# AOS55/exorl

Measured on AMD Instinct MI355X. Metric: gradient-steps/sec TD3+BC walker_walk batch=1024, higher is better.
Workload: dtype bf16x3

## Files before the change

exorl_amd/csrc/fused.hip:

```cpp
#include "kernels.h"

namespace exorl {

constexpr int MAX_IN = 256;
constexpr float LN_EPS2 = 1e-5f;

constexpr int TF_ROWS = 8;
constexpr int TF_LDS_FLOATS = 35 * 1024;

__device__ __forceinline__ float tanh_fast(float x) {
    const float e = __expf(2.0f * x);
    return 1.0f - 2.0f * __frcp_rn(1.0f + e);
}

template <bool FAST>
__global__ __launch_bounds__(512) void trunk_fwd_kernel(const float* __restrict__ x, int64_t ldx,
                                                        const float* __restrict__ W0T, const float* __restrict__ b0,
                                                        const float* __restrict__ gain, const float* __restrict__ beta,
                                                        float* __restrict__ h, float* __restrict__ xhat,
                                                        float* __restrict__ rstd, unsigned short* __restrict__ hb,
                                                        unsigned short* __restrict__ xhb, int rows, int in_dim, int H,
                                                        int64_t astride, int64_t pstride, int64_t tstride, int TF_KC) {
    extern __shared__ __attribute__((aligned(16))) float smem[];
    float* ws = smem;
// ... 956 lines not shown
        float4 v;
        v.x = av.x > 0.f ? sacc.x : 0.f; v.y = av.y > 0.f ? sacc.y : 0.f;
        v.z = av.z > 0.f ? sacc.z : 0.f; v.w = av.w > 0.f ? sacc.w : 0.f;
        if (dz) reinterpret_cast<float4*>(dz + o)[c4] = v;
        if (dzb) reinterpret_cast<ushort4*>(dzb + o)[c4] = bf16_bits4(v);
        if (dzl) reinterpret_cast<ushort4*>(dzl + o)[c4] = bf16_lo_bits4(v);
        pb.x += v.x; pb.y += v.y; pb.z += v.z; pb.w += v.w;
    }
    if (want_params) {
#pragma unroll
        for (int j = 0; j < NO; ++j)
            if (j < nout) reinterpret_cast<float4*>(Pn + (int64_t)j * H)[c4] = pw[j];
        reinterpret_cast<float4*>(Pn + (int64_t)nout * H)[c4] = pb;
    }
}

int head_bwd(const DoutSpec& dspec, const float* W, const float* a, float* dz, const Planes& dzq, float* P, int rows,
             int H, int nout, int nets, int64_t astride, int64_t pstride, int want_params, hipStream_t s, bool metrics) {
    unsigned short *dz_bf16 = dzq.hi, *dz_lo = dzq.lo;
    EXORL_REQUIRE(nout >= 1 && nout <= 16 && H % 4 == 0 && H <= 1024, "head_bwd: nout=%d H=%d unsupported", nout, H);
    dim3 grid(cdiv(rows, HB_ROWS), nets);
    if (metrics) {
        EXORL_REQUIRE(dspec.mode == EXORL_DOUT_ACTOR_MU && dspec.kind == EXORL_AGENT_TD3_BC && nets == 1 && dspec.bc_part,
                      "head_bwd: the metrics variant is TD3+BC's actor gradient on one net");
        if (nout == 1) hipLaunchKernelGGL((head_bwd_kernel<1, true>), grid, dim3(256), 0, s, dspec, W, a, dz, dz_bf16, P, rows, H, nout, astride, pstride, want_params, dz_lo);
        else if (nout <= 8) hipLaunchKernelGGL((head_bwd_kernel<8, true>), grid, dim3(256), 0, s, dspec, W, a, dz, dz_bf16, P, rows, H, nout, astride, pstride, want_params, dz_lo);
        else hipLaunchKernelGGL((head_bwd_kernel<16, true>), grid, dim3(256), 0, s, dspec, W, a, dz, dz_bf16, P, rows, H, nout, astride, pstride, want_params, dz_lo);
    } else if (nout == 1) hipLaunchKernelGGL((head_bwd_kernel<1>), grid, dim3(256), 0, s, dspec, W, a, dz, dz_bf16, P, rows, H, nout, astride, pstride, want_params, dz_lo);
    else if (nout <= 8) hipLaunchKernelGGL((head_bwd_kernel<8>), grid, dim3(256), 0, s, dspec, W, a, dz, dz_bf16, P, rows, H, nout, astride, pstride, want_params, dz_lo);
    else hipLaunchKernelGGL((head_bwd_kernel<16>), grid, dim3(256), 0, s, dspec, W, a, dz, dz_bf16, P, rows, H, nout, astride, pstride, want_params, dz_lo);
    EXORL_LAUNCH_CHECK();
    return 0;
}
__global__ __launch_bounds__(256) void head_bwd_wide_kernel(const DoutSpec dspec, const float* __restrict__ W,
                                                            const float* __restrict__ a, float* __restrict__ dz,
                                                            unsigned short* __restrict__ dzb, float* __restrict__ P, int rows, int H,
                                                            int nout, int64_t astride, int64_t pstride, int want_params,
                                                            unsigned short* __restrict__ dzl) {
    __shared__ float ds[HB_ROWS * 32];
    const int net = blockIdx.z;
    const int row0 = blockIdx.y * HB_ROWS;
    const int c = blockIdx.x * 256 + threadIdx.x;
    {
        const int r = threadIdx.x >> 5, j = threadIdx.x & 31;
        ds[threadIdx.x] = (row0 + r < rows && j < nout) ? dout_value(dspec, net, row0 + r, j, rows, nout) : 0.f;
    }
    __syncthreads();
    const int64_t nh = (int64_t)(nout + 1) * H + 32;
    float* Pn = P ? P + ((int64_t)net * gridDim.y + blockIdx.y) * nh : nullptr;
    if (want_params && blockIdx.x == 0 && threadIdx.x < nout) {
        float sj = 0.f;
        for (int r = 0; r < HB_ROWS; ++r) sj += ds[r * 32 + threadIdx.x];
        Pn[(int64_t)(nout + 1) * H + threadIdx.x] = sj;
    }
    if (c >= H) return;
    float w[32], pw[32];
#pragma unroll
    for (int j = 0; j < 32; ++j) {
        w[j] = j < nout ? W[net * pstride + (int64_t)j * H + c] : 0.f;
        pw[j] = 0.f;
    }
    float pb = 0.f;
    const int nr = rows - row0 < HB_ROWS ? rows - row0 : HB_ROWS;
    for (int r = 0; r < nr; ++r) {
        const int64_t o = net * astride + (int64_t)(row0 + r) * H + c;
        const float av = a[o];
        float sacc = 0.f;
#pragma unroll
        for (int j = 0; j < 32; ++j) {
            const float d = ds[r * 32 + j];
            sacc += d * w[j];
            pw[j] += d * av;
        }
        const float v = av > 0.f ? sacc : 0.f;
        if (dz) dz[o] = v;
        if (dzb) dzb[o] = bf16_bits(v);
        if (dzl) dzl[o] = bf16_lo_bits(v);
        pb += v;
    }
    if (want_params) {
#pragma unroll
        for (int j = 0; j < 32; ++j)
            if (j < nout) Pn[(int64_t)j * H + c] = pw[j];
        Pn[(int64_t)nout * H + c] = pb;
    }
}

int head_bwd_wide(const DoutSpec& dspec, const float* W, const float* a, float* dz, const Planes& dzq, float* P, int rows, int H,
                  int nout, int64_t astride, int64_t pstride, int want_params, hipStream_t s) {
    unsigned short *dz_bf16 = dzq.hi, *dz_lo = dzq.lo;
    EXORL_REQUIRE(nout > 16 && nout <= 32, "head_bwd_wide: nout=%d out of range", nout);
    hipLaunchKernelGGL(head_bwd_wide_kernel, dim3(cdiv(H, 256), cdiv(rows, HB_ROWS), 1), dim3(256), 0, s, dspec, W, a, dz, dz_bf16, P, rows,
                       H, nout, astride, pstride, want_params, dz_lo);
    EXORL_LAUNCH_CHECK();
    return 0;
}

int head_chunks(int rows) { return cdiv(rows, HB_ROWS); }

constexpr int QH_ROWS = 4;
template <int MODE, bool TP, bool MET = false>
__global__ __launch_bounds__(256) void qhead_kernel(const QHeadArgs g) {
    __shared__ float part[4][4 * QH_ROWS];
    __shared__ float dq[2 * QH_ROWS];
    __shared__ float met[6 * QH_ROWS];
    const int row0 = blockIdx.x * QH_ROWS;
    const int c4 = threadIdx.x, H = g.H, H4 = H >> 2;
    const int lane = threadIdx.x & 63, wave = threadIdx.x >> 6;
    const int nr = g.rows - row0 < QH_ROWS ? g.rows - row0 : QH_ROWS;
    constexpr int nn = (MODE == 0 && !TP) ? 4 : 2;
    const bool on = c4 < H4;
    float4 avs[2][QH_ROWS];
    float4 w[2];
    float dots[4 * QH_ROWS];
    float4 wvs[nn], ts[nn][QH_ROWS];
    {
        const int cc = on ? c4 : 0;
#pragma unroll
        for (int n = 0; n < nn; ++n) {
            wvs[n] = reinterpret_cast<const float4*>(g.W[n])[cc];
#pragma unroll
            for (int r = 0; r < QH_ROWS; ++r) ts[n][r] = reinterpret_cast<const float4*>(g.a[n] + (int64_t)(row0 + (r < nr ? r : 0)) * H)[cc];
        }
    }
#pragma unroll
    for (int n = 0; n < 4; ++n) {
        if (n >= nn) {
#pragma unroll
            for (int r = 0; r < QH_ROWS; ++r) dots[n * QH_ROWS + r] = 0.f;
            continue;
        }
        const float4 wv = on ? wvs[n < nn ? n : 0] : make_float4(0.f, 0.f, 0.f, 0.f);
        if (n < 2) w[n] = wv;
#pragma unroll
        for (int r = 0; r < QH_ROWS; ++r) {
            const float4 t = (on && r < nr) ? ts[n < nn ? n : 0][r] : make_float4(0.f, 0.f, 0.f, 0.f);
            dots[n * QH_ROWS + r] = (t.x * wv.x + t.y * wv.y) + (t.z * wv.z + t.w * wv.w);
            if (n < 2) avs[n][r] = t;
        }
    }
#pragma unroll
    for (int i = 0; i < 4 * QH_ROWS; ++i) {
        const float v = wave_sum(dots[i]);
        if (lane == 0) part[wave][i] = v;
    }
    __syncthreads();
    if (threadIdx.x < 4 * QH_ROWS) {
        const int n = threadIdx.x / QH_ROWS, r = threadIdx.x % QH_ROWS;
        if (n < nn && r < nr) {
            const float v = ((part[0][threadIdx.x] + part[1][threadIdx.x]) + (part[2][threadIdx.x] + part[3][threadIdx.x])) + g.b[n][0];
            part[0][threadIdx.x] = v;
            (n < 2 ? g.q : g.tq)[(int64_t)(n & 1) * g.rows + row0 + r] = v;
        } else if (TP && MODE == 0 && n >= 2 && r < nr) {
            const float* tp = g.tpart[n - 2] + (int64_t)(row0 + r) * g.tslots;
            float v = 0.f;
            for (int j = 0; j < g.tslots; ++j) v += tp[j];
            v += g.b[n][0];
            part[0][threadIdx.x] = v;
            g.tq[(int64_t)(n & 1) * g.rows + row0 + r] = v;
        }
    }
    __syncthreads();
    if (threadIdx.x < 2 * QH_ROWS) {
        const int n = threadIdx.x / QH_ROWS, r = threadIdx.x % QH_ROWS;
        float d = 0.f, m_r = 0.f, m_y = 0.f, m_q = 0.f, m_e = 0.f;
        if (r < nr) {
            const float q1 = part[0][r], q2 = part[0][QH_ROWS + r];
            if (MODE == 0) {
                const float rw = g.reward[row0 + r];
                const float y = rw + g.discount[row0 + r] * fminf(part[0][2 * QH_ROWS + r], part[0][3 * QH_ROWS + r]);
                d = 2.0f * ((n == 0 ? q1 : q2) - y) * g.inv_bg;
                m_r = rw; m_y = y; m_q = n == 0 ? q1 : q2; m_e = (m_q - y) * (m_q - y);
            } else {
                const float w1 = q1 < q2 ? 1.0f : (q1 == q2 ? 0.5f : 0.0f);
                d = -g.inv_bg * (n == 0 ? w1 : 1.0f - w1);
            }
        }
        dq[threadIdx.x] = d;
        if (MODE == 0 && MET) {
            if (n == 0) { met[r] = m_r; met[QH_ROWS + r] = m_y; }
            met[(2 + n) * QH_ROWS + r] = m_q;
            met[(4 + n) * QH_ROWS + r] = m_e;
        }
    }
    if (MODE == 1 && threadIdx.x == 0) {
        float sa = 0.f, sm = 0.f;
        for (int r = 0; r < nr; ++r) { const float m = fminf(part[0][r], part[0][QH_ROWS + r]); sa += fabsf(m); sm += m; }
        g.abs_part[2 * blockIdx.x] = sa;
        g.abs_part[2 * blockIdx.x + 1] = sm;
    }
    __syncthreads();
    if (MODE == 0 && MET && threadIdx.x < 6) {
        float sk = 0.f;
        for (int r = 0; r < QH_ROWS; ++r) sk += met[threadIdx.x * QH_ROWS + r];
        g.abs_part[6 * blockIdx.x + threadIdx.x] = sk;
    }
    const int64_t nh = 2 * (int64_t)H + 16;
#pragma unroll
    for (int n = 0; n < 2; ++n) {
        float* Pn = g.P ? g.P + ((int64_t)n * gridDim.x + blockIdx.x) * nh : nullptr;
        if (Pn && threadIdx.x == 0) {
            float sj = 0.f;
            for (int r = 0; r < QH_ROWS; ++r) sj += dq[n * QH_ROWS + r];
            Pn[2 * (int64_t)H] = sj;
        }
        if (!on) continue;
        float4 pw = make_float4(0.f, 0.f, 0.f, 0.f), pb = make_float4(0.f, 0.f, 0.f, 0.f);
#pragma unroll
        for (int r = 0; r < QH_ROWS; ++r) {
            if (r >= nr) break;
            const float d = dq[n * QH_ROWS + r];
            const float4 av = avs[n][r];
            pw.x += d * av.x; pw.y += d * av.y; pw.z += d * av.z; pw.w += d * av.w;
            float4 v;
            v.x = av.x > 0.f ? d * w[n].x : 0.f; v.y = av.y > 0.f ? d * w[n].y : 0.f;
            v.z = av.z > 0.f ? d * w[n].z : 0.f; v.w = av.w > 0.f ? d * w[n].w : 0.f;
            const int64_t o = n * g.act + (int64_t)(row0 + r) * H;
            if (g.dz) reinterpret_cast<float4*>(g.dz + o)[c4] = v;
            if (g.dzb) reinterpret_cast<ushort4*>(g.dzb + o)[c4] = bf16_bits4(v);
            if (g.dzl) reinterpret_cast<ushort4*>(g.dzl + o)[c4] = bf16_lo_bits4(v);
            pb.x += v.x; pb.y += v.y; pb.z += v.z; pb.w += v.w;
        }
        if (Pn) {
            reinterpret_cast<float4*>(Pn)[c4] = pw;
            reinterpret_cast<float4*>(Pn + H)[c4] = pb;
        }
    }
}

int qhead_chunks(int rows) { return cdiv(rows, QH_ROWS); }

int qhead(const QHeadArgs& q, hipStream_t s, bool metrics) {
    EXORL_REQUIRE(q.H % 4 == 0 && q.H <= 1024 && q.rows > 0 && (q.mode == 0 || q.mode == 1), "qhead: unsupported H=%d rows=%d", q.H, q.rows);
    if (q.mode == 0 && metrics && q.tpart[0]) hipLaunchKernelGGL((qhead_kernel<0, true, true>), dim3(cdiv(q.rows, QH_ROWS)), dim3(256), 0, s, q);
    else if (q.mode == 0 && metrics) hipLaunchKernelGGL((qhead_kernel<0, false, true>), dim3(cdiv(q.rows, QH_ROWS)), dim3(256), 0, s, q);
    else if (q.mode == 0 && q.tpart[0]) hipLaunchKernelGGL((qhead_kernel<0, true>), dim3(cdiv(q.rows, QH_ROWS)), dim3(256), 0, s, q);
    else if (q.mode == 0) hipLaunchKernelGGL((qhead_kernel<0, false>), dim3(cdiv(q.rows, QH_ROWS)), dim3(256), 0, s, q);
    else hipLaunchKernelGGL((qhead_kernel<1, false>), dim3(cdiv(q.rows, QH_ROWS)), dim3(256), 0, s, q);
    EXORL_LAUNCH_CHECK();
    return 0;
}

__global__ __launch_bounds__(256) void finalize_grads_kernel(FinalizeArgs f) {
    const int H = f.H;
    const int64_t nh = (int64_t)(f.nout + 1) * H + (f.nout > 16 ? 32 : 16);
    const int64_t nt = 3 * (int64_t)H;
    const int64_t nw = (int64_t)f.in_dim * H;
    const int64_t total = f.n_heads * nh + f.n_trunks * (nt + nw);
    for (int64_t i = blockIdx.x * (int64_t)blockDim.x + threadIdx.x; i < total; i += (int64_t)gridDim.x * blockDim.x) {
        if (i < f.n_heads * nh) {
            const int net = (int)(i / nh);
            const int64_t e = i % nh;
            const int64_t j = e / H;
            if (j > f.nout && e - (int64_t)(f.nout + 1) * H >= f.nout) continue;
            const float sacc = chunk_sum(f.Ph + (int64_t)net * f.head_chunks * nh + e, f.head_chunks, nh);
            float* Gn = f.G + net * f.head_stride;
            if (j < f.nout) Gn[f.gW2 + e] = sacc;
            else if (j == f.nout) Gn[f.gb1 + (e - (int64_t)f.nout * H)] = sacc;
            else Gn[f.gb2 + (e - (int64_t)(f.nout + 1) * H)] = sacc;
        } else {
            const int64_t ii = i - f.n_heads * nh;
            const int net = (int)(ii / (nt + nw));
            const int64_t e = ii % (nt + nw);
            float* Gn = f.G + net * f.trunk_stride;
            if (e < nt) {
                const float sacc = chunk_sum(f.Pt + (int64_t)net * f.trunk_chunks * nt + e, f.trunk_chunks, nt);
                const int seg = (int)(e / H), c = (int)(e % H);
                if (seg == 0) Gn[f.gg + c] = sacc;
                else if (seg == 1) Gn[f.gbeta + c] = sacc;
                else Gn[f.gb0 + c] = sacc;
            } else {
                const int64_t ew = e - nt;
                const float sacc = chunk_sum(f.Pw + (int64_t)net * f.w_chunks * nw + ew, f.w_chunks, nw);
                const int k = (int)(ew / H), c = (int)(ew % H);
                Gn[f.gW0 + (int64_t)c * f.in_dim + k] = sacc;
            }
        }
    }
}

__device__ __forceinline__ void step_small(const FusedAdamArgs& a, const AdamConst& c, int64_t gi, float grad, float& pnew, float& tnew) {
    a.g[gi] = grad;
    float p = a.p[gi], m = a.m[gi], v = a.v[gi];
    adam_elem(p, grad, m, v, c);
    a.p[gi] = p; a.m[gi] = m; a.v[gi] = v;
    pnew = p; tnew = 0.f;
    if (a.target) {
        tnew = polyak(p, a.target[gi], c.tau, c.one_minus_tau);
        a.target[gi] = tnew;
    }
}

__device__ __forceinline__ float4 ld4(const float* p, int64_t i4) { return reinterpret_cast<const float4*>(p)[i4]; }
__device__ __forceinline__ void st4(float* p, int64_t i4, const float4& v) { reinterpret_cast<float4*>(p)[i4] = v; }

struct FlatShadows {
    int n_trunks, n_heads, in_dim, H;
    int64_t w0_off[2], w1_off[2];
    float* w0t; unsigned short *w1b, *w0b;
    float* t_w0t; unsigned short *t_w1b, *t_w0b;
    unsigned short *w1l, *w0l, *t_w1l, *t_w0l;
};

__global__ __launch_bounds__(256) void finalize_adam_kernel(FinalizeArgs f, FusedAdamArgs a, FlatShadows sh, int nb_fin) {
    const AdamConst c = *a.c;
    if (a.bump && blockIdx.x == 0 && threadIdx.x == 0) *a.bump += 1ull;
    const int H = f.H;
    if ((int)blockIdx.x >= nb_fin) {
        const int64_t hh8 = (int64_t)H * H / 8, n8 = a.n_heads * hh8;
        for (int64_t i = (int64_t)(blockIdx.x - nb_fin) * blockDim.x + threadIdx.x; i < n8; i += (int64_t)(gridDim.x - nb_fin) * blockDim.x) {
            const int t = (int)(i / hh8);
            const int64_t e8 = i % hh8, gi4 = a.w1_off[t] / 4 + 2 * e8;
            float4 pv[2], gv[2], mv[2], vv[2], tv[2];
#pragma unroll
            for (int u = 0; u < 2; ++u) {
                pv[u] = ld4(a.p, gi4 + u);
                gv[u] = ld4(a.g, gi4 + u);
                mv[u] = ld4(a.m, gi4 + u);
                vv[u] = ld4(a.v, gi4 + u);
                tv[u] = a.target ? ld4(a.target, gi4 + u) : make_float4(0.f, 0.f, 0.f, 0.f);
            }
            ushort4 bh[2], bl[2], th[2], tl[2];
#pragma unroll
            for (int u = 0; u < 2; ++u) {
                adam_elem(pv[u].x, gv[u].x, mv[u].x, vv[u].x, c); adam_elem(pv[u].y, gv[u].y, mv[u].y, vv[u].y, c);
                adam_elem(pv[u].z, gv[u].z, mv[u].z, vv[u].z, c); adam_elem(pv[u].w, gv[u].w, mv[u].w, vv[u].w, c);
                st4(a.p, gi4 + u, pv[u]);
                st4(a.m, gi4 + u, mv[u]);
                st4(a.v, gi4 + u, vv[u]);
                bh[u] = bf16_bits4(pv[u]); bl[u] = bf16_lo_bits4(pv[u]);
                if (a.target) {
                    tv[u].x = polyak(pv[u].x, tv[u].x, c.tau, c.one_minus_tau); tv[u].y = polyak(pv[u].y, tv[u].y, c.tau, c.one_minus_tau);
                    tv[u].z = polyak(pv[u].z, tv[u].z, c.tau, c.one_minus_tau); tv[u].w = polyak(pv[u].w, tv[u].w, c.tau, c.one_minus_tau);
                    st4(a.target, gi4 + u, tv[u]);
                    th[u] = bf16_bits4(tv[u]); tl[u] = bf16_lo_bits4(tv[u]);
                }
            }
            auto pack = [](const ushort4& x, const ushort4& y) {
                uint4 r;
                r.x = x.x | ((unsigned)x.y << 16); r.y = x.z | ((unsigned)x.w << 16); r.z = y.x | ((unsigned)y.y << 16); r.w = y.z | ((unsigned)y.w << 16);
                return r;
            };
            if (sh.w1b) reinterpret_cast<uint4*>(sh.w1b + (int64_t)t * H * H)[e8] = pack(bh[0], bh[1]);
            if (sh.w1l) reinterpret_cast<uint4*>(sh.w1l + (int64_t)t * H * H)[e8] = pack(bl[0], bl[1]);
            if (a.target) {
                if (sh.t_w1b) reinterpret_cast<uint4*>(sh.t_w1b + (int64_t)t * H * H)[e8] = pack(th[0], th[1]);
                if (sh.t_w1l) reinterpret_cast<uint4*>(sh.t_w1l + (int64_t)t * H * H)[e8] = pack(tl[0], tl[1]);
            }
        }
        return;
    }
    const int64_t nh = (int64_t)(f.nout + 1) * H + (f.nout > 16 ? 32 : 16);
    const int64_t nt = 3 * (int64_t)H;
    const int64_t nw = (int64_t)f.in_dim * H;
    const int64_t total = f.n_heads * nh + f.n_trunks * (nt + nw);
    const int64_t Kp = (f.in_dim + 31) / 32 * 32;
    for (int64_t i = blockIdx.x * (int64_t)blockDim.x + threadIdx.x; i < total; i += (int64_t)nb_fin * blockDim.x) {
        float pn, tn;
        if (i < f.n_heads * nh) {
            const int net = (int)(i / nh);
            const int64_t e = i % nh;
            const int64_t j = e / H;
            if (j > f.nout && e - (int64_t)(f.nout + 1) * H >= f.nout) continue;
            const float sacc = chunk_sum(f.Ph + (int64_t)net * f.head_chunks * nh + e, f.head_chunks, nh);
            const int64_t base = net * f.head_stride;
            const int64_t gi = base + (j < f.nout ? f.gW2 + e : (j == f.nout ? f.gb1 + (e - (int64_t)f.nout * H) : f.gb2 + (e - (int64_t)(f.nout + 1) * H)));
            step_small(a, c, gi, sacc, pn, tn);
        } else {
            const int64_t ii = i - f.n_heads * nh;
            const int net = (int)(ii / (nt + nw));
            const int64_t e = ii % (nt + nw);
            const int64_t base = net * f.trunk_stride;
            if (e < nt) {
                const float sacc = chunk_sum(f.Pt + (int64_t)net * f.trunk_chunks * nt + e, f.trunk_chunks, nt);
                const int seg = (int)(e / H), cc = (int)(e % H);
                step_small(a, c, base + (seg == 0 ? f.gg : (seg == 1 ? f.gbeta : f.gb0)) + cc, sacc, pn, tn);
            } else {
                const int64_t ew = e - nt;
                const float sacc = chunk_sum(f.Pw + (int64_t)net * f.w_chunks * nw + ew, f.w_chunks, nw);
                const int k = (int)(ew / H), cc = (int)(ew % H);
                step_small(a, c, base + f.gW0 + (int64_t)cc * f.in_dim + k, sacc, pn, tn);
                sh.w0t[net * nw + (int64_t)k * H + cc] = pn;
                if (sh.w0b) sh.w0b[(int64_t)net * H * Kp + (int64_t)cc * Kp + k] = bf16_bits(pn);
                if (sh.w0l) sh.w0l[(int64_t)net * H * Kp + (int64_t)cc * Kp + k] = bf16_lo_bits(pn);
                if (a.target && sh.t_w0t) {
                    sh.t_w0t[net * nw + (int64_t)k * H + cc] = tn;
                    if (sh.t_w0b) sh.t_w0b[(int64_t)net * H * Kp + (int64_t)cc * Kp + k] = bf16_bits(tn);
                    if (sh.t_w0l) sh.t_w0l[(int64_t)net * H * Kp + (int64_t)cc * Kp + k] = bf16_lo_bits(tn);
                }
            }
        }
    }
}

int finalize_adam(const FinalizeArgs& f, const FusedAdamArgs& a, const ShadowSpec& sh, hipStream_t s) {
    EXORL_REQUIRE(sh.H % 4 == 0 && a.n_heads >= 1 && a.n_heads <= 2, "finalize_adam: unsupported geometry");
    const int H = sh.H;
    const int64_t total = f.n_heads * ((int64_t)(f.nout + 1) * f.H + (f.nout > 16 ? 32 : 16)) + f.n_trunks * (int64_t)(3 + f.in_dim) * f.H;
    const int nb_fin = cdiv(total, 256);
    int nb_w1 = cdiv((int64_t)a.n_heads * H * H / 8, 256);
    if (nb_w1 > 2048) nb_w1 = 2048;
    FlatShadows flat{};
    flat.n_trunks = sh.n_trunks; flat.n_heads = sh.n_heads; flat.in_dim = sh.in_dim; flat.H = sh.H;
    for (int i = 0; i < 2; ++i) { flat.w0_off[i] = sh.w0_off[i]; flat.w1_off[i] = sh.w1_off[i]; }
    flat.w0t = sh.own.w0t;      flat.w1b = sh.own.w1.hi;      flat.w1l = sh.own.w1.lo;      flat.w0b = sh.own.w0.hi;      flat.w0l = sh.own.w0.lo;
    flat.t_w0t = sh.target.w0t; flat.t_w1b = sh.target.w1.hi; flat.t_w1l = sh.target.w1.lo; flat.t_w0b = sh.target.w0.hi; flat.t_w0l = sh.target.w0.lo;
    hipLaunchKernelGGL(finalize_adam_kernel, dim3(nb_fin + nb_w1), dim3(256), 0, s, f, a, flat, nb_fin);
    EXORL_LAUNCH_CHECK();
    return 0;
}

int finalize_grads(const FinalizeArgs& f, hipStream_t s) {
    const int64_t total = f.n_heads * ((int64_t)(f.nout + 1) * f.H + (f.nout > 16 ? 32 : 16)) + f.n_trunks * (int64_t)(3 + f.in_dim) * f.H;
    hipLaunchKernelGGL(finalize_grads_kernel, dim3(cdiv(total, 256)), dim3(256), 0, s, f);
    EXORL_LAUNCH_CHECK();
    return 0;
}

}
```

exorl_amd/csrc/kernels.h:

```cpp
#pragma once
#include <vector>

#include "numerics.h"

namespace exorl {

struct TensorDesc { int64_t off, rows, cols; };

struct SimpleCarver {
    float* base; int64_t off = 0;
    explicit SimpleCarver(float* b) : base(b) {}
    float* take(int64_t n) { float* p = base ? base + off : nullptr; off += round_up(n, 64); return p; }
};

struct Planes {
    unsigned short *hi = nullptr, *mid = nullptr, *lo = nullptr;
    __host__ __device__ Planes at(int64_t off) const { return Planes{hi ? hi + off : nullptr, mid ? mid + off : nullptr, lo ? lo + off : nullptr}; }
    __host__ __device__ explicit operator bool() const { return hi != nullptr; }
};

struct GemmProblem {
    const float* A;
    const float* B;
    float* C;
    const float* bias;
    int M, N, K;
    int64_t lda, ldb, ldc;
};
int gemm_grouped(int precision, int a_layout, int b_layout, const GemmProblem* probs, int count, bool relu,
                 bool accumulate, hipStream_t s);
void gemm_planes_capture(bool allow, size_t* probe);
int gemm_planes_reserve(size_t bytes);

struct Gemm16Problem {
    const unsigned short* A;
    const unsigned short* B;
    float* C;
    const float* bias;
    int M, N, K;
    int64_t lda, ldb, ldc;
    const unsigned short* A_lo = nullptr;
    const unsigned short* B_lo = nullptr;
    const float* head_w = nullptr;
    float* head_part = nullptr;
    int n_store = 0;
    const unsigned short* A_mid = nullptr;
    const unsigned short* B_mid = nullptr;
};
int to_planes3(const float* src, int64_t ld, int rows, int cols, unsigned short* hi, unsigned short* mid, unsigned short* lo, int rows_p, int cols_p,
               int nb, int64_t src_stride, int64_t dst_stride, hipStream_t s);
int gemm16_head_slots(const Gemm16Problem* probs, int count);
int gemm16_grouped(int a_layout, int b_layout, const Gemm16Problem* probs, int count, bool relu, bool accumulate, hipStream_t s);
int gemm16_grouped_mixed(const int* a_layouts, const Gemm16Problem* probs, int count, hipStream_t s);

int ln_tanh_fwd(const float* z, const float* gain, const float* beta, float* h, float* xhat, float* rstd,
                int rows, int H, int nets, int64_t astride, int64_t pstride, hipStream_t s);
int ln_tanh_bwd(const float* dh, const float* h, const float* xhat, const float* rstd, const float* gain, float* dz,
                int rows, int H, int nets, int64_t astride, int64_t pstride, hipStream_t s);
int ln_param_grad(const float* dh, const float* h, const float* xhat, float* dgain, float* dbeta,
                  int rows, int H, int nets, int64_t astride, int64_t pstride, hipStream_t s);
int colsum(const float* x, float* out, int rows, int cols, int nets, int64_t astride, int64_t pstride, hipStream_t s);
int relu_bwd_colsum(float* x, const float* act, float* out, int rows, int cols, hipStream_t s);
int linear_splitk(int prec, const float* x, int64_t ldx, const float* W, const float* b, float* out, int rows, int F, int K, float* scratch,
                  int splits, hipStream_t s);
int head_fwd(const float* a, const float* W, const float* b, float* out, int rows, int H, int nout, int tanh_out,
             int nets, int64_t astride, int64_t pstride, int64_t ostride, hipStream_t s);
int head_bwd_dx(const float* dout, const float* W, const float* a, float* dz, int rows, int H, int nout,
                int nets, int64_t astride, int64_t pstride, int64_t dstride, hipStream_t s);
int head_bwd_params(const float* dout, const float* a, const float* dz, float* dW, float* db_hidden, float* db_out,
                    int rows, int H, int nout, int nets, int64_t astride, int64_t pstride, int64_t dstride, hipStream_t s);

int trunk_fwd(const float* x, int64_t ldx, const float* W0T, const float* b0, const float* gain, const float* beta,
              float* h, float* xhat, float* rstd, unsigned short* h_bf16, unsigned short* xhat_bf16, int rows, int in_dim,
              int H, int nets, int64_t astride, int64_t pstride, int64_t tstride, hipStream_t s);
struct TrunkItem { const float* x; const unsigned short* W0b; const float *b0, *gain, *beta; float* rstd; unsigned short *hb, *xhb;
                   const unsigned short* W0l; unsigned short *hl, *xhl; };
struct TrunkBatch { TrunkItem it[4]; };
int trunk_fwd16_batch(const TrunkBatch& tb, int count, int64_t ldx, int rows, int in_dim, int H, hipStream_t s);
struct HeadItem { const float* a; const float* W; const float* b; float* out; };
struct HeadBatch { HeadItem it[4]; };
int head_fwd1_batch(const HeadBatch& hb, int count, int rows, int H, hipStream_t s);
bool trunk_fwd16_supported(int H);
int trunk_fwd16(const float* x, int64_t ldx, const Planes& W0q, const float* b0, const float* gain, const float* beta, float* rstd,
                const Planes& hq, const Planes& xhatq, int rows, int in_dim, int H, int nets, int64_t astride, int64_t pstride, hipStream_t s);
int ln_bwd(float* dh, const float* h, const float* xhat, const Planes& hq, const Planes& xhatq, const float* rstd, const float* gain, float* P,
           int rows, int H, int nets, int64_t astride, int64_t pstride, int want_params, hipStream_t s, const float* w0t, int64_t tstride,
           float* dx, int dx_cols, const float* beta);
int trunk_chunks(int rows);
int64_t knn_scratch_floats(int n_src, int n_tgt);
int knn_topk(const float* src, int n_src, const float* tgt, int n_tgt, int dim, int k, float* out, float* d2, hipStream_t s);
int outer_reduce(const float* u, int64_t ldu, int J, const float* v, float* P, int rows, int H, int nets, int64_t vstride,
                 hipStream_t s);
int outer_chunks(int rows);
struct SampleSpec {
    const float* stddev_ptr;
    const float *noise_c, *noise_a;
    uint64_t seed;
    const uint64_t* counter_ptr;
    float stddev, clip;
    float *dst_next, *dst_pi;
    int64_t dst_ld;
    int B;
};
int head_fwd4(const float* a, const float* W, const float* b, float* out, int rows, int H, int nout, int tanh_out,
              int nets, int64_t astride, int64_t pstride, int64_t ostride, hipStream_t s, const SampleSpec* sample = nullptr);
#define EXORL_DOUT_BUFFER   0
#define EXORL_DOUT_TD       1
#define EXORL_DOUT_ACTOR_Q  2
#define EXORL_DOUT_CQL_ACTOR 4
#define EXORL_DOUT_ACTOR_MU 3
struct DoutSpec {
    int mode;
    union {
        const float* buf;
        float* bc_part;
    };
    const float *q, *tq, *reward, *discount;
    const float* stats;
    const float *da, *mu, *a_data;
    const float* w;
    const float *raw, *z;
    const float* alpha_ptr;
    uint64_t seed, counter; const uint64_t* counter_ptr;
    const float* task;
    int64_t task_ld;
    const float* lam_parts;
    int lam_chunks;
    int da_nets;
    int kind;
    int use_lambda;
    float inv_bg, alpha, stddev;
    const float* stddev_ptr;
};
int head_bwd(const DoutSpec& dspec, const float* W, const float* a, float* dz, const Planes& dzq, float* P, int rows,
             int H, int nout, int nets, int64_t astride, int64_t pstride, int want_params, hipStream_t s, bool metrics = false);
int head_chunks(int rows);
int tune_variant();
constexpr int TUNE_CONV_WGRAD_TILE = 64;
constexpr int TUNE_ACT_GENERIC = 256;
constexpr int TUNE_CONV_PER_IMAGE = 8388608;
constexpr int TUNE_ADAPTER_PADDED = 134217728;
constexpr int TUNE_CONV_STRIP = 1073741824;
int prec_override_mask();
struct QHeadArgs {
    const float* a[4];
    const float* W[4];
    const float* b[4];
    float *q, *tq;
    const float *reward, *discount;
    float* dz; unsigned short* dzb; unsigned short* dzl; int64_t act;
    float* P;
    float* abs_part;
    const float* tpart[2];
    int tslots;
    int rows, H, mode;
    float inv_bg;
};
int qhead(const QHeadArgs& q, hipStream_t s, bool metrics = false);
int qhead_chunks(int rows);
__device__ __forceinline__ float chunk_sum(const float* __restrict__ p, int n, int64_t stride) {
    float acc = 0.f;
    int ch = 0;
    if (n > 1024) {
        for (; ch + 32 <= n; ch += 32) {
            float t[32], sub = 0.f;
#pragma unroll
            for (int q = 0; q < 32; ++q) t[q] = p[(int64_t)(ch + q) * stride];
#pragma unroll
            for (int q = 0; q < 32; ++q) sub += t[q];
            acc += sub;
        }
    }
    for (; ch + 32 <= n; ch += 32) {
        float t[32];
#pragma unroll
        for (int q = 0; q < 32; ++q) t[q] = p[(int64_t)(ch + q) * stride];
#pragma unroll
        for (int q = 0; q < 32; ++q) acc += t[q];
    }
    for (; ch + 16 <= n; ch += 16) {
        float t[16];
#pragma unroll
        for (int q = 0; q < 16; ++q) t[q] = p[(int64_t)(ch + q) * stride];
#pragma unroll
        for (int q = 0; q < 16; ++q) acc += t[q];
    }
    for (; ch < n; ++ch) acc += p[(int64_t)ch * stride];
    return acc;
}

struct FinalizeArgs {
    const float* Ph; int head_chunks; int n_heads; int64_t head_stride;
    int64_t gW2, gb1, gb2;
    const float* Pt; int trunk_chunks; int n_trunks; int64_t trunk_stride;
    const float* Pw; int w_chunks;
    int64_t gW0, gb0, gg, gbeta;
    int H, nout, in_dim;
    float* G;
};
int finalize_grads(const FinalizeArgs& f, hipStream_t s);

__device__ __forceinline__ float polyak(float p, float t, float tau, float one_minus_tau) {
#pragma clang fp contract(off)
    const float a = tau * p;
    const float b = one_minus_tau * t;
    return a + b;
}
struct AdamConst;
struct FusedAdamArgs {
    float *p, *g, *m, *v, *target;
    const AdamConst* c;
    int n_heads; int64_t w1_off[2];
    unsigned long long* bump;
};
struct ShadowSpec;
int finalize_adam(const FinalizeArgs& f, const FusedAdamArgs& a, const ShadowSpec& sh, hipStream_t s);

struct WeightImages { float* w0t = nullptr; Planes w1, w0; };
__host__ __device__ inline int64_t w0_kp(int64_t in_dim) { return (in_dim + 31) / 32 * 32; }
__host__ __device__ inline int64_t w0t_size(int64_t in_dim, int64_t H) { return in_dim * H; }
__host__ __device__ inline int64_t w0_plane_size(int64_t in_dim, int64_t H) { return H * w0_kp(in_dim); }
__host__ __device__ inline int64_t w1_plane_size(int64_t H) { return H * H; }
__host__ __device__ inline int64_t w0t_index(int64_t trunk, int64_t k, int64_t c, int64_t in_dim, int64_t H) { return trunk * w0t_size(in_dim, H) + k * H + c; }
__host__ __device__ inline int64_t w0_plane_index(int64_t trunk, int64_t c, int64_t k, int64_t in_dim, int64_t H) {
    return trunk * w0_plane_size(in_dim, H) + c * w0_kp(in_dim) + k;
}
struct ShadowSpec {
    int n_trunks, n_heads, in_dim, H;
    int64_t w0_off[2], w1_off[2];
    WeightImages own, target;
};
int refresh_shadows(const float* p, int64_t n, const ShadowSpec& sh, bool target, hipStream_t s);

struct NoiseSpec {
    const float* buf;
    uint64_t seed;
    uint64_t counter;
    const uint64_t* counter_ptr;
};

struct AdamConst {
    float one_minus_b1, b2, one_minus_b2, bc2_sqrt, eps, neg_step_size, tau, one_minus_tau;
};

__device__ __forceinline__ void adam_elem(float& p, float g, float& m, float& v, const AdamConst& c) {
#pragma clang fp contract(off)
    m = m + c.one_minus_b1 * (g - m);
    v = v * c.b2 + (c.one_minus_b2 * g) * g;
    const float denom = sqrtf(v) / c.bc2_sqrt + c.eps;
    p = p + (c.neg_step_size * m) / denom;
}

struct StepState {
    uint64_t replay_counter;
    uint64_t noise_counter;
    long long t_actor, t_critic;
    double b1t, b2t_actor_unused, b1t_c, b2t_c;
    double b2t;
    AdamConst actor, critic;
    double lr, b1, b2, eps, tau;
    int has_critic;
    float stddev;
};
int step_begin(StepState* st, int advance_replay, hipStream_t s);

struct IntrStepState {
    uint64_t counter;
    uint64_t draw_counter;
    long long t;
    long long queue_ptr;
    long long qrow0;
    int queue_size, num_protos;
    int draws;
    double b1t, b2t;
    double b1, b2, eps;
    double lr[3];
    AdamConst c[3];
};
constexpr int ACT_FAST_ROWS = 2;
struct ActFast {
    const float *x_dev, *x_host;
    const float *w0t, *P;
    int64_t b0, g, beta, W1, b1, W2, b2;
    float* part; unsigned int* ticket;
    const float *noise_dev, *noise_host;
    uint64_t seed, counter;
    float* out;
    float stddev;
    int rows, in_dim, H, nout, eval_mode;
    int first_relu = 0; int64_t W0 = 0;
};
bool act_fast_supported(int rows, int in_dim, int H, int nout);
int act_fast(const ActFast& f, hipStream_t s);
int trunk_one(const float* x, const float* meta, const float* W, const float* b, const float* gain, const float* beta, float* part, unsigned int* ticket,
              float* out, int R, int M, int F, hipStream_t s);
int reduce_pairs(const float* parts, int chunks, float* out, hipStream_t s);
struct MetricsWindowArgs {
    const float *crit_part, *abs_part, *bc_part;
    int q_chunks, bc_chunks;
    int fused;
    int kind, act_dim, ent_from_std;
    float inv_bg, alpha;
    const float* stddev;
    float* metrics;
    double* sums; long long* steps;
};
int metrics_window(const MetricsWindowArgs& w, hipStream_t s);
int set_device_float(float* dst, float value, hipStream_t s);
int set_device_u64(uint64_t* dst, uint64_t value, hipStream_t s);

__host__ __device__ inline void fill_adam_const(AdamConst& c, double b1t, double b2t, double lr, double b1, double b2, double eps, double tau) {
    const double bc1 = 1.0 - b1t;
    const double bc2 = 1.0 - b2t;
    c.one_minus_b1 = (float)(1.0 - b1);
    c.b2 = (float)b2;
    c.one_minus_b2 = (float)(1.0 - b2);
    c.bc2_sqrt = (float)sqrt(bc2);
    c.eps = (float)eps;
    c.neg_step_size = (float)(-(lr / bc1));
    c.tau = (float)tau;
    c.one_minus_tau = (float)(1.0 - tau);
}

__device__ inline void step_begin_device(StepState* st, int advance_replay) {
    if (advance_replay) st->replay_counter += 1;
    st->noise_counter += 2;
    st->t_actor += 1;
    st->b1t *= st->b1;
    st->b2t *= st->b2;
    fill_adam_const(st->actor, st->b1t, st->b2t, st->lr, st->b1, st->b2, st->eps, 0.0);
    if (st->has_critic) {
        st->t_critic += 1;
        st->b1t_c *= st->b1;
        st->b2t_c *= st->b2;
        fill_adam_const(st->critic, st->b1t_c, st->b2t_c, st->lr, st->b1, st->b2, st->eps, st->tau);
    }
}


__device__ inline void intr_step_begin_device(IntrStepState* st) {
    st->t += 1;
    st->b1t *= st->b1;
    st->b2t *= st->b2;
    for (int i = 0; i < 3; ++i) fill_adam_const(st->c[i], st->b1t, st->b2t, st->lr[i], st->b1, st->b2, st->eps, 0.0);
    st->draw_counter = st->counter;
    st->counter += (uint64_t)st->draws;
    st->qrow0 = st->queue_ptr;
    if (st->queue_size > 0) st->queue_ptr = (st->queue_ptr + st->num_protos) % st->queue_size;
}

int prepare_inputs(const float* obs, const float* action, const float* next_obs, float* xa, float* xc_cur,
                   float* xc_next, float* xc_pi, int B, int O, int A, int has_critic, StepState* st, int advance_replay,
                   hipStream_t s);
int sample_actions2(const float* mu2, const float* noise_c, const float* noise_a, uint64_t seed, const uint64_t* counter_ptr,
                    float stddev, float clip, float* dst_next, float* dst_pi, int64_t dst_ld, int B, int A, hipStream_t s,
                    const float* stddev_ptr = nullptr);
int sample_action(const float* mu, NoiseSpec noise, float stddev, float clip, int use_clip, float* dst, int64_t dst_ld,
                  int B, int A, float* logprob_sum, hipStream_t s, const float* stddev_ptr = nullptr, int world_size = 1);
struct CqlNoise {
    const float *z_next, *u_rand, *z_cur, *z_nxt, *z_actor;
    uint64_t seed;
    const uint64_t* counter_ptr;
};
struct CqlScalars {
    float log_alpha, m, v, alpha;
};
int cql_build_inputs(const float* obs, const float* action, const float* raw2, CqlNoise nz, float* xc_next, float* x_all, int B,
                     int O, int A, int n, hipStream_t s);
int cql_critic_dq(const float* q_all, const float* tq, const float* reward, const float* discount, float* dq_all, float* metrics,
                  int B, int n, float cql_alpha, float inv_bg, hipStream_t s, CqlScalars* lag = nullptr, const AdamConst* c_dev = nullptr,
                  float target_penalty = 0.f,
                  int mode = 0, float* gsum = nullptr);
int cql_actor_sample(const float* raw_obs, CqlNoise nz, float* xc_pi, int64_t ld, float* stats, int B, int O, int A, hipStream_t s);
int cql_alpha_step(CqlScalars* sc, const float* stats, const AdamConst* c_dev, float* metrics, int B, int A, float inv_bg, const float* q,
                   hipStream_t s);
int cql_act(const float* raw, const float* noise, uint64_t seed, uint64_t counter, int eval_mode, float* out, int rows, int A, hipStream_t s);
int head_bwd_wide(const DoutSpec& dspec, const float* W, const float* a, float* dz, const Planes& dzq, float* P, int rows, int H,
                  int nout, int64_t astride, int64_t pstride, int want_params, hipStream_t s);

int repeat_sample(const float* obs, const float* mu, const float* noise, uint64_t seed, const uint64_t* counter_ptr, uint64_t counter,
                  float stddev, float clip, float* xc_rep, int B, int O, int A, int n, hipStream_t s, const float* stddev_ptr = nullptr);
int crr_weights(const float* q_rep, const float* q_data, float* w, int B, int n, int weight_func, hipStream_t s);
int critic_loss(const float* q, const float* tq, const float* reward, const float* discount, float* dq,
                float* metrics, int B, float inv_bg, hipStream_t s);
int actor_stats(const float* q, float* stats, int B, hipStream_t s);
int sf_q(const float* feat, const float* task, int64_t task_ld, float* q, int B, int sf, int nets, hipStream_t s);
int actor_dq(const float* q, const float* stats, float* dq, int B, float inv_bg, float alpha, int use_lambda,
             hipStream_t s);
int actor_dmu(const float* da, int64_t da_ld, int da_nets, int64_t da_net_stride, const float* mu, const float* a_data, const float* reward, const float* w, float* dpre, float* stats,
              float* metrics, int B, int A, float inv_bg, float alpha, int kind, float stddev, hipStream_t s, const float* stddev_ptr = nullptr);

int adam_step(float* p, const float* g, float* m, float* v, int64_t n, float lr, float b1, float b2, float eps,
              int64_t t, float* target, float tau, hipStream_t s);
int soft_update(const float* p, float* target, int64_t n, float tau, hipStream_t s);
int adam_step_dev(float* p, const float* g, float* m, float* v, int64_t n, const AdamConst* c_dev, float* target,
                  const ShadowSpec* shadows, hipStream_t s, uint64_t* bump = nullptr);

struct Lin { int in, out; int64_t W, b; };
struct Mlp {
    std::vector<Lin> L;
    bool relu_last = false;
    std::vector<float*> act, dact;
};
int mlp_forward(const Mlp& m, const float* P, const float* x, int64_t ldx, int rows, int prec, hipStream_t s);
int mlp_backward(const Mlp& m, const float* P, float* G, const float* x, int64_t ldx, int rows, float* dx, int prec, hipStream_t s);
int mlp_forward_many(const Mlp* nets, int n, const float* P, const float* x, int64_t ldx, int rows, int prec, hipStream_t s);
int mlp_backward_many(const Mlp* nets, int n, const float* P, float* G, const float* x, int64_t ldx, int rows, int prec, hipStream_t s, float* dx);
int launch_concat(const float* a, int64_t lda, int ca, const float* b, int64_t ldb, int cb, float* dst, int rows, hipStream_t s);

int intr_graph_prepare(exorl_intr* it, const exorl_intr_batch* b, hipStream_t capture);
int intr_graph_capture(exorl_intr* it, const exorl_intr_batch* b, hipStream_t capture);
int intr_graph_before_launch(exorl_intr* it, hipStream_t s);
void intr_graph_after_launch(exorl_intr* it);
void intr_graph_release(exorl_intr* it);
int copy_meta_columns(const float* obs, float* next_obs, int64_t ld, int rows, int O, int M, hipStream_t s);

struct StageOut {
    float *xa, *xc_cur, *xc_next, *xc_pi;
    int O, A, B, has_critic;
    StepState* st;
};
int replay_sample_impl(exorl_replay* r, int32_t batch, int32_t nstep, float gamma, int32_t sampler,
                       const int32_t* pairs_host, const exorl_batch_out* out, int32_t* pairs_out_host, hipStream_t s,
                       const uint64_t* dev_counter, const StageOut* stage = nullptr);
int replay_obs_bytes(exorl_replay* r);
int replay_frame_stack(exorl_replay* r);
void replay_dims(exorl_replay* r, int* act_dim, int* meta_dim);
int comm_allreduce_sum(exorl_comm* c, float* buf, int64_t n, hipStream_t s);
int comm_nranks(const exorl_comm* c);

uint64_t replay_philox_counter(exorl_replay* r);
uint64_t replay_weights_epoch(exorl_replay* r);
int replay_prepare(exorl_replay* r, int32_t batch, int32_t nstep, hipStream_t s);
void replay_advance_philox(exorl_replay* r, uint64_t n);

}
```

Before: 3300.

## Tile chunk reductions across workgroups and software-pipeline W1 Adam loads

```diff
diff --git a/exorl_amd/csrc/fused.hip b/exorl_amd/csrc/fused.hip
--- a/exorl_amd/csrc/fused.hip
+++ b/exorl_amd/csrc/fused.hip
@@ -1282,93 +1282,106 @@
     unsigned short *w1l, *w0l, *t_w1l, *t_w0l;
 };
 
-__global__ __launch_bounds__(256) void finalize_adam_kernel(FinalizeArgs f, FusedAdamArgs a, FlatShadows sh, int nb_fin) {
+constexpr int W1_WG_PER_CU = 2;
+
+struct W1Group { float4 p, g, m, v, t; };
+
+template <bool TGT> __device__ __forceinline__ void w1_load(W1Group& r, const FusedAdamArgs& a, int64_t i, int64_t n4, int64_t hh4) {
+    i = i < n4 ? i : n4 - 1;
+    const bool second = i >= hh4;
+    const int64_t gi4 = (second ? a.w1_off[1] : a.w1_off[0]) / 4 + (second ? i - hh4 : i);
+    r.p = ld4(a.p, gi4);
+    r.g = ld4(a.g, gi4);
+    r.m = ld4(a.m, gi4);
+    r.v = ld4(a.v, gi4);
+    if (TGT) r.t = ld4(a.target, gi4);
+}
+
+template <bool TGT> __device__ __forceinline__ void w1_finish(W1Group& r, const FusedAdamArgs& a, const FlatShadows& sh, const AdamConst& c, int64_t i,
+                                                              int64_t n4, int64_t hh4) {
+    if (i >= n4) return;
+    const bool second = i >= hh4;
+    const int64_t e4 = second ? i - hh4 : i, gi4 = (second ? a.w1_off[1] : a.w1_off[0]) / 4 + e4, plane = second ? 4 * hh4 : 0;
+    adam_elem(r.p.x, r.g.x, r.m.x, r.v.x, c); adam_elem(r.p.y, r.g.y, r.m.y, r.v.y, c);
+    adam_elem(r.p.z, r.g.z, r.m.z, r.v.z, c); adam_elem(r.p.w, r.g.w, r.m.w, r.v.w, c);
+    st4(a.p, gi4, r.p);
+    st4(a.m, gi4, r.m);
+    st4(a.v, gi4, r.v);
+    if (sh.w1b) reinterpret_cast<ushort4*>(sh.w1b + plane)[e4] = bf16_bits4(r.p);
+    if (sh.w1l) reinterpret_cast<ushort4*>(sh.w1l + plane)[e4] = bf16_lo_bits4(r.p);
+    if (TGT) {
+        float4& tv = r.t;
+        tv.x = polyak(r.p.x, tv.x, c.tau, c.one_minus_tau); tv.y = polyak(r.p.y, tv.y, c.tau, c.one_minus_tau);
+        tv.z = polyak(r.p.z, tv.z, c.tau, c.one_minus_tau); tv.w = polyak(r.p.w, tv.w, c.tau, c.one_minus_tau);
+        st4(a.target, gi4, tv);
+        if (sh.t_w1b) reinterpret_cast<ushort4*>(sh.t_w1b + plane)[e4] = bf16_bits4(tv);
+        if (sh.t_w1l) reinterpret_cast<ushort4*>(sh.t_w1l + plane)[e4] = bf16_lo_bits4(tv);
+    }
+}
+
+template <bool TGT>
+__global__ __launch_bounds__(256, 4) void finalize_adam_kernel(FinalizeArgs f, FusedAdamArgs a, FlatShadows sh, int nb_fin) {
     const AdamConst c = *a.c;
     if (a.bump && blockIdx.x == 0 && threadIdx.x == 0) *a.bump += 1ull;
     const int H = f.H;
     if ((int)blockIdx.x >= nb_fin) {
-        const int64_t hh8 = (int64_t)H * H / 8, n8 = a.n_heads * hh8;
-        for (int64_t i = (int64_t)(blockIdx.x - nb_fin) * blockDim.x + threadIdx.x; i < n8; i += (int64_t)(gridDim.x - nb_fin) * blockDim.x) {
-            const int t = (int)(i / hh8);
-            const int64_t e8 = i % hh8, gi4 = a.w1_off[t] / 4 + 2 * e8;
-            float4 pv[2], gv[2], mv[2], vv[2], tv[2];
-#pragma unroll
-            for (int u = 0; u < 2; ++u) {
-                pv[u] = ld4(a.p, gi4 + u);
-                gv[u] = ld4(a.g, gi4 + u);
-                mv[u] = ld4(a.m, gi4 + u);
-                vv[u] = ld4(a.v, gi4 + u);
-                tv[u] = a.target ? ld4(a.target, gi4 + u) : make_float4(0.f, 0.f, 0.f, 0.f);
-            }
-            ushort4 bh[2], bl[2], th[2], tl[2];
-#pragma unroll
-            for (int u = 0; u < 2; ++u) {
-                adam_elem(pv[u].x, gv[u].x, mv[u].x, vv[u].x, c); adam_elem(pv[u].y, gv[u].y, mv[u].y, vv[u].y, c);
-                adam_elem(pv[u].z, gv[u].z, mv[u].z, vv[u].z, c); adam_elem(pv[u].w, gv[u].w, mv[u].w, vv[u].w, c);
-                st4(a.p, gi4 + u, pv[u]);
-                st4(a.m, gi4 + u, mv[u]);
-                st4(a.v, gi4 + u, vv[u]);
-                bh[u] = bf16_bits4(pv[u]); bl[u] = bf16_lo_bits4(pv[u]);
-                if (a.target) {
-                    tv[u].x = polyak(pv[u].x, tv[u].x, c.tau, c.one_minus_tau); tv[u].y = polyak(pv[u].y, tv[u].y, c.tau, c.one_minus_tau);
-                    tv[u].z = polyak(pv[u].z, tv[u].z, c.tau, c.one_minus_tau); tv[u].w = polyak(pv[u].w, tv[u].w, c.tau, c.one_minus_tau);
-                    st4(a.target, gi4 + u, tv[u]);
-                    th[u] = bf16_bits4(tv[u]); tl[u] = bf16_lo_bits4(tv[u]);
-                }
-            }
-            auto pack = [](const ushort4& x, const ushort4& y) {
-                uint4 r;
-                r.x = x.x | ((unsigned)x.y << 16); r.y = x.z | ((unsigned)x.w << 16); r.z = y.x | ((unsigned)y.y << 16); r.w = y.z | ((unsigned)y.w << 16);
-                return r;
-            };
-            if (sh.w1b) reinterpret_cast<uint4*>(sh.w1b + (int64_t)t * H * H)[e8] = pack(bh[0], bh[1]);
-            if (sh.w1l) reinterpret_cast<uint4*>(sh.w1l + (int64_t)t * H * H)[e8] = pack(bl[0], bl[1]);
-            if (a.target) {
-                if (sh.t_w1b) reinterpret_cast<uint4*>(sh.t_w1b + (int64_t)t * H * H)[e8] = pack(th[0], th[1]);
-                if (sh.t_w1l) reinterpret_cast<uint4*>(sh.t_w1l + (int64_t)t * H * H)[e8] = pack(tl[0], tl[1]);
-            }
+        const int64_t hh4 = (int64_t)H * H / 4, n4 = a.n_heads * hh4;
+        const int64_t step = (int64_t)(gridDim.x - nb_fin) * 256, i0 = (int64_t)((int)blockIdx.x - nb_fin) * 256 + threadIdx.x;
+        const int rounds = (int)((n4 + step - 1) / step);
+        W1Group r0, r1;
+        w1_load<TGT>(r0, a, i0, n4, hh4);
+        for (int it = 0; it < rounds; it += 2) {
+            const int64_t i = i0 + it * step;
+            w1_load<TGT>(r1, a, i + step, n4, hh4);
+            w1_finish<TGT>(r0, a, sh, c, i, n4, hh4);
+            w1_load<TGT>(r0, a, i + 2 * step, n4, hh4);
+            w1_finish<TGT>(r1, a, sh, c, i + step, n4, hh4);
         }
         return;
     }
+    __shared__ float tile[CS_SLAB][CS_TILE];
     const int64_t nh = (int64_t)(f.nout + 1) * H + (f.nout > 16 ? 32 : 16);
     const int64_t nt = 3 * (int64_t)H;
     const int64_t nw = (int64_t)f.in_dim * H;
-    const int64_t total = f.n_heads * nh + f.n_trunks * (nt + nw);
-    const int64_t Kp = (f.in_dim + 31) / 32 * 32;
-    for (int64_t i = blockIdx.x * (int64_t)blockDim.x + threadIdx.x; i < total; i += (int64_t)nb_fin * blockDim.x) {
+    const int tiles_h = (int)((nh + CS_TILE - 1) / CS_TILE), tiles_t = (int)((nt + CS_TILE - 1) / CS_TILE);
+    const int nb_tiles = f.n_heads * tiles_h + f.n_trunks * tiles_t;
+    if ((int)blockIdx.x < nb_tiles) {
         float pn, tn;
-        if (i < f.n_heads * nh) {
-            const int net = (int)(i / nh);
-            const int64_t e = i % nh;
+        if ((int)blockIdx.x < f.n_heads * tiles_h) {
+            const int net = blockIdx.x / tiles_h;
+            const int64_t e0 = (int64_t)(blockIdx.x % tiles_h) * CS_TILE, e = e0 + threadIdx.x;
+            const float sacc = chunk_sum_tile(f.Ph + (int64_t)net * f.head_chunks * nh, f.head_chunks, nh, e0, nh, tile);
+            if (threadIdx.x >= CS_TILE || e >= nh) return;
             const int64_t j = e / H;
-            if (j > f.nout && e - (int64_t)(f.nout + 1) * H >= f.nout) continue;
-            const float sacc = chunk_sum(f.Ph + (int64_t)net * f.head_chunks * nh + e, f.head_chunks, nh);
+            if (j > f.nout && e - (int64_t)(f.nout + 1) * H >= f.nout) return;
             const int64_t base = net * f.head_stride;
             const int64_t gi = base + (j < f.nout ? f.gW2 + e : (j == f.nout ? f.gb1 + (e - (int64_t)f.nout * H) : f.gb2 + (e - (int64_t)(f.nout + 1) * H)));
             step_small(a, c, gi, sacc, pn, tn);
         } else {
-            const int64_t ii = i - f.n_heads * nh;
-            const int net = (int)(ii / (nt + nw));
-            const int64_t e = ii % (nt + nw);
-            const int64_t base = net * f.trunk_stride;
-            if (e < nt) {
-                const float sacc = chunk_sum(f.Pt + (int64_t)net * f.trunk_chunks * nt + e, f.trunk_chunks, nt);
-                const int seg = (int)(e / H), cc = (int)(e % H);
-                step_small(a, c, base + (seg == 0 ? f.gg : (seg == 1 ? f.gbeta : f.gb0)) + cc, sacc, pn, tn);
-            } else {
-                const int64_t ew = e - nt;
-                const float sacc = chunk_sum(f.Pw + (int64_t)net * f.w_chunks * nw + ew, f.w_chunks, nw);
-                const int k = (int)(ew / H), cc = (int)(ew % H);
-                step_small(a, c, base + f.gW0 + (int64_t)cc * f.in_dim + k, sacc, pn, tn);
-                sh.w0t[net * nw + (int64_t)k * H + cc] = pn;
-                if (sh.w0b) sh.w0b[(int64_t)net * H * Kp + (int64_t)cc * Kp + k] = bf16_bits(pn);
-                if (sh.w0l) sh.w0l[(int64_t)net * H * Kp + (int64_t)cc * Kp + k] = bf16_lo_bits(pn);
-                if (a.target && sh.t_w0t) {
-                    sh.t_w0t[net * nw + (int64_t)k * H + cc] = tn;
-                    if (sh.t_w0b) sh.t_w0b[(int64_t)net * H * Kp + (int64_t)cc * Kp + k] = bf16_bits(tn);
-                    if (sh.t_w0l) sh.t_w0l[(int64_t)net * H * Kp + (int64_t)cc * Kp + k] = bf16_lo_bits(tn);
-                }
-            }
+            const int b = blockIdx.x - f.n_heads * tiles_h, net = b / tiles_t;
+            const int64_t e0 = (int64_t)(b % tiles_t) * CS_TILE, e = e0 + threadIdx.x;
+            const float sacc = chunk_sum_tile(f.Pt + (int64_t)net * f.trunk_chunks * nt, f.trunk_chunks, nt, e0, nt, tile);
+            if (threadIdx.x >= CS_TILE || e >= nt) return;
+            const int seg = (int)(e / H), cc = (int)(e % H);
+            step_small(a, c, net * f.trunk_stride + (seg == 0 ? f.gg : (seg == 1 ? f.gbeta : f.gb0)) + cc, sacc, pn, tn);
+        }
+        return;
+    }
+    const int64_t Kp = (f.in_dim + 31) / 32 * 32;
+    for (int64_t i = (int64_t)((int)blockIdx.x - nb_tiles) * blockDim.x + threadIdx.x; i < f.n_trunks * nw; i += (int64_t)(nb_fin - nb_tiles) * blockDim.x) {
+        float pn, tn;
+        const int net = (int)(i / nw);
+        const int64_t ew = i % nw;
+        const float sacc = chunk_sum(f.Pw + (int64_t)net * f.w_chunks * nw + ew, f.w_chunks, nw);
+        const int k = (int)(ew / H), cc = (int)(ew % H);
+        step_small(a, c, net * f.trunk_stride + f.gW0 + (int64_t)cc * f.in_dim + k, sacc, pn, tn);
+        sh.w0t[net * nw + (int64_t)k * H + cc] = pn;
+        if (sh.w0b) sh.w0b[(int64_t)net * H * Kp + (int64_t)cc * Kp + k] = bf16_bits(pn);
+        if (sh.w0l) sh.w0l[(int64_t)net * H * Kp + (int64_t)cc * Kp + k] = bf16_lo_bits(pn);
+        if (a.target && sh.t_w0t) {
+            sh.t_w0t[net * nw + (int64_t)k * H + cc] = tn;
+            if (sh.t_w0b) sh.t_w0b[(int64_t)net * H * Kp + (int64_t)cc * Kp + k] = bf16_bits(tn);
+            if (sh.t_w0l) sh.t_w0l[(int64_t)net * H * Kp + (int64_t)cc * Kp + k] = bf16_lo_bits(tn);
         }
     }
 }
@@ -1376,16 +1389,25 @@
 int finalize_adam(const FinalizeArgs& f, const FusedAdamArgs& a, const ShadowSpec& sh, hipStream_t s) {
     EXORL_REQUIRE(sh.H % 4 == 0 && a.n_heads >= 1 && a.n_heads <= 2, "finalize_adam: unsupported geometry");
     const int H = sh.H;
-    const int64_t total = f.n_heads * ((int64_t)(f.nout + 1) * f.H + (f.nout > 16 ? 32 : 16)) + f.n_trunks * (int64_t)(3 + f.in_dim) * f.H;
-    const int nb_fin = cdiv(total, 256);
-    int nb_w1 = cdiv((int64_t)a.n_heads * H * H / 8, 256);
-    if (nb_w1 > 2048) nb_w1 = 2048;
+    const int64_t nh = (int64_t)(f.nout + 1) * f.H + (f.nout > 16 ? 32 : 16), nt = 3 * (int64_t)f.H;
+    const int nb_fin = f.n_heads * cdiv(nh, CS_TILE) + f.n_trunks * cdiv(nt, CS_TILE) + cdiv(f.n_trunks * (int64_t)f.in_dim * f.H, 256);
+    static int cus = 0;
+    if (cus == 0) {
+        int dev = 0, n = 0;
+        EXORL_CHECK_HIP(hipGetDevice(&dev));
+        EXORL_CHECK_HIP(hipDeviceGetAttribute(&n, hipDeviceAttributeMultiprocessorCount, dev));
+        EXORL_REQUIRE(n > 0, "finalize_adam: device reports %d compute units", n);
+        cus = n;
+    }
+    int nb_w1 = cdiv((int64_t)a.n_heads * H * H / 4, 256);
+    if (nb_w1 > W1_WG_PER_CU * cus) nb_w1 = W1_WG_PER_CU * cus;
     FlatShadows flat{};
     flat.n_trunks = sh.n_trunks; flat.n_heads = sh.n_heads; flat.in_dim = sh.in_dim; flat.H = sh.H;
     for (int i = 0; i < 2; ++i) { flat.w0_off[i] = sh.w0_off[i]; flat.w1_off[i] = sh.w1_off[i]; }
     flat.w0t = sh.own.w0t;      flat.w1b = sh.own.w1.hi;      flat.w1l = sh.own.w1.lo;      flat.w0b = sh.own.w0.hi;      flat.w0l = sh.own.w0.lo;
     flat.t_w0t = sh.target.w0t; flat.t_w1b = sh.target.w1.hi; flat.t_w1l = sh.target.w1.lo; flat.t_w0b = sh.target.w0.hi; flat.t_w0l = sh.target.w0.lo;
-    hipLaunchKernelGGL(finalize_adam_kernel, dim3(nb_fin + nb_w1), dim3(256), 0, s, f, a, flat, nb_fin);
+    if (a.target) hipLaunchKernelGGL(finalize_adam_kernel<true>, dim3(nb_fin + nb_w1), dim3(256), 0, s, f, a, flat, nb_fin);
+    else hipLaunchKernelGGL(finalize_adam_kernel<false>, dim3(nb_fin + nb_w1), dim3(256), 0, s, f, a, flat, nb_fin);
     EXORL_LAUNCH_CHECK();
     return 0;
 }
diff --git a/exorl_amd/csrc/kernels.h b/exorl_amd/csrc/kernels.h
--- a/exorl_amd/csrc/kernels.h
+++ b/exorl_amd/csrc/kernels.h
@@ -189,6 +189,39 @@
     return acc;
 }
 
+constexpr int CS_TILE = 64, CS_SLAB = 128;
+__device__ __forceinline__ float chunk_sum_tile(const float* __restrict__ p, int n, int64_t stride, int64_t e0, int64_t ne, float (*tile)[CS_TILE]) {
+    const int l = threadIdx.x % CS_TILE, r = threadIdx.x / CS_TILE;
+    const int64_t e = e0 + l < ne ? e0 + l : ne - 1;
+    float acc = 0.f;
+    for (int s0 = 0; s0 < n; s0 += CS_SLAB) {
+        float t[CS_SLAB / 4];
+#pragma unroll
+        for (int q = 0; q < CS_SLAB / 4; ++q) {
+            const int ch = s0 + r + 4 * q;
+            t[q] = p[(int64_t)(ch < n ? ch : n - 1) * stride + e];
+        }
+#pragma unroll
+        for (int q = 0; q < CS_SLAB / 4; ++q) tile[r + 4 * q][l] = t[q];
+        __syncthreads();
+        if (threadIdx.x < CS_TILE) {
+            const int m = n - s0 < CS_SLAB ? n - s0 : CS_SLAB;
+            int ch = 0;
+            if (n > 1024) {
+                for (; ch + 32 <= m; ch += 32) {
+                    float sub = 0.f;
+#pragma unroll
+                    for (int q = 0; q < 32; ++q) sub += tile[ch + q][l];
+                    acc += sub;
+                }
+            }
+            for (; ch < m; ++ch) acc += tile[ch][l];
+        }
+        __syncthreads();
+    }
+    return acc;
+}
+
 struct FinalizeArgs {
     const float* Ph; int head_chunks; int n_heads; int64_t head_stride;
     int64_t gW2, gb1, gb2;
```

Result: no change. 3317, median of 3 (+0.5%).
